# caesar-one/audio-classification-using-a-deep-cnn-combined-with-multi-level-attention

Measured on NVIDIA B200. Metric: 10s-clip audio->logits clips/sec, higher is better.
Workload: dtype fp16

## Files before the change

### audio-classification-using-a-deep-cnn-combined-with-multi-level-attention_b200/b200/_lib.py

```python
from __future__ import annotations

import ctypes as C
import os

_HERE = os.path.dirname(os.path.abspath(__file__))
LIB_PATH = os.environ.get("VMB_LIB") or os.path.join(_HERE, "libvggish_mla_b200.so")

_c_p = C.c_void_p
_ll = C.c_longlong
_int = C.c_int
_sz = C.c_size_t

SIGNATURES = {
    "vmb_last_error": (C.c_char_p, []),
    "vmb_abi_version": (_int, []),
    "vmb_device_arch": (_int, [_int]),
    "vmb_launch_count": (_ll, []),
    "vmb_igemm_pair_enable": (_int, [_int]),
    "vmb_igemm_halo_enable": (_int, [_int]),
    "vmb_mla_fuse_enable": (_int, [_int]),
    "vmb_profile_enable": (_int, [_int]),
    "vmb_profile_collect": (_int, [_c_p, _c_p, _int]),
    "vmb_num_frames": (_ll, [_ll]),
    "vmb_num_examples": (_ll, [_ll]),
    "vmb_logmel": (_int, [_c_p, _ll, _ll, _ll, _ll, _c_p, _c_p]),
    "vmb_logmel_pcm16": (_int, [_c_p, _ll, _ll, _ll, _ll, _c_p, _c_p]),
    "vmb_logmel_cudacore": (_int, [_c_p, _ll, _ll, _ll, _ll, _c_p, _c_p]),
    "vmb_stft_magnitude": (_int, [_c_p, _ll, _c_p, _c_p]),
    "vmb_spec_tiles": (_int, [_c_p, _ll, _int, _int, _int, _c_p, _c_p]),
    "vmb_front_end_tables": (_int, [_c_p, _c_p]),
    "vmb_conv1_relu_pool": (_int, [_c_p, _c_p, _c_p, _c_p, _ll, _c_p]),
    "vmb_conv1_relu_pool_ex": (_int, [_c_p, _c_p, _c_p, _c_p, _ll, _int, _c_p]),
    "vmb_conv1_relu_pool_cudacore": (_int, [_c_p, _c_p, _c_p, _c_p, _ll, _c_p]),
    "vmb_conv3x3_relu": (_int, [_c_p, _c_p, _c_p, _c_p, _ll, _int, _int, _int, _int, _int, _c_p]),
    "vmb_conv3x3_relu_ex": (_int, [_c_p, _c_p, _c_p, _c_p, _ll, _int, _int, _int, _int, _int, _int, _c_p]),
    "vmb_linear_ex": (_int, [_c_p, _c_p, _c_p, _c_p, _int, _int, _ll, _int, _int, _int, _c_p]),
    "vmb_linear": (_int, [_c_p, _c_p, _c_p, _c_p, _int, _int, _ll, _int, _int, _c_p]),
    "vmb_postprocess": (_int, [_c_p, _c_p, _c_p, _c_p, _c_p, _ll, _c_p]),
    "vmb_vggish_create": (_int, [C.POINTER(_c_p), C.POINTER(_c_p), C.POINTER(_c_p), C.POINTER(_c_p),
                                 C.POINTER(_c_p), _c_p]),
    "vmb_vggish_create_ex": (_int, [C.POINTER(_c_p), C.POINTER(_c_p), C.POINTER(_c_p), C.POINTER(_c_p),
                                    C.POINTER(_c_p), _int, _c_p]),
    "vmb_vggish_precision": (_int, [_c_p]),
    "vmb_vggish_saturation": (_int, [_c_p, _int]),
    "vmb_vggish_handle_workspace_bytes": (_sz, [_c_p, _ll]),
    "vmb_vggish_destroy": (None, [_c_p]),
    "vmb_vggish_workspace_bytes": (_sz, [_ll]),
    "vmb_vggish_forward": (_int, [_c_p, _c_p, _ll, _c_p, _c_p, _c_p, _sz, _c_p]),
    "vmb_vggish_fc_train_workspace_bytes": (_sz, [_ll]),
    "vmb_vggish_fc_grad_count": (_ll, []),
    "vmb_vggish_refresh_fc": (_int, [_c_p, C.POINTER(_c_p), C.POINTER(_c_p), _c_p]),
    "vmb_vggish_forward_train": (_int, [_c_p, _c_p, _ll, _c_p, _c_p, _sz, _c_p]),
# ... 79 lines not shown
```

### audio-classification-using-a-deep-cnn-combined-with-multi-level-attention_b200/csrc/api.cu

```cuda
#include "../../include/vggish_mla_b200.h"

#include <cuda_runtime.h>

#include <cstdarg>
#include <cstdio>
#include <cstring>

#include "igemm_sm100.cuh"
#include "kernels.cuh"

namespace {
thread_local char g_api_err[768] = "";

int fail(const char* fmt, ...) {
  va_list ap;
  va_start(ap, fmt);
  vsnprintf(g_api_err, sizeof g_api_err, fmt, ap);
  va_end(ap);
  return 1;
}
int fail_from(const char* where, const char* inner) { return fail("%s: %s", where, inner); }

cudaStream_t S(void* s) { return static_cast<cudaStream_t>(s); }
}

namespace vmb {
void set_api_error(const char* msg) { snprintf(g_api_err, sizeof g_api_err, "%s", msg); }
}

extern "C" {

const char* vmb_last_error(void) { return g_api_err; }
int vmb_abi_version(void) { return 2; }

int vmb_device_arch(int device) {
  int major = 0, minor = 0;
  if (cudaDeviceGetAttribute(&major, cudaDevAttrComputeCapabilityMajor, device) != cudaSuccess ||
      cudaDeviceGetAttribute(&minor, cudaDevAttrComputeCapabilityMinor, device) != cudaSuccess) {
    fail("vmb_device_arch: no CUDA device %d (%s)", device, cudaGetErrorString(cudaGetLastError()));
    return -1;
  }
  return major * 10 + minor;
}

int vmb_igemm_pair_enable(int on) { return vmb::igemm_set_pair(on); }
int vmb_igemm_halo_enable(int on) { return vmb::igemm_set_halo(on); }

long long vmb_num_frames(long long n_samples) {
  const long long d = n_samples - 400;
  long long q = d / 160;
  if (d % 160 != 0 && d < 0) --q;
  return 1 + q;
}

long long vmb_num_examples(long long n_samples) {
  const long long f = vmb_num_frames(n_samples);
  if (f < 96) return f < 0 ? -1 : 0;
  return 1 + (f - 96) / 96;
}

static int logmel_common(const char* who, bool tensor_core, const float* wave, long long n_clips,
                         long long samples_per_clip, long long clip_stride, long long frames_out, float* logmel,
                         void* stream) {
  if (n_clips < 0 || frames_out < 0) return fail("%s: negative size", who);
  const long long nf = vmb_num_frames(samples_per_clip);
  if (nf < 1) return fail("%s: %lld samples is shorter than one 400-sample window", who, samples_per_clip);
  if (frames_out > nf) return fail("%s: frames_out %lld > available frames %lld", who, frames_out, nf);
  if (clip_stride < samples_per_clip) return fail("%s: clip_stride < samples_per_clip", who);
  if (n_clips == 0 || frames_out == 0) return 0;
  if (!wave || !logmel) return fail("%s: null pointer", who);
  const int rc = tensor_core
                     ? vmb::logmel_tc_forward(wave, n_clips, samples_per_clip, clip_stride, frames_out, logmel, S(stream))
                     : vmb::logmel_forward(wave, n_clips, samples_per_clip, clip_stride, frames_out, logmel, S(stream));
  if (rc) return fail_from(who, vmb::kernels_last_error());
  return 0;
}

int vmb_logmel(const float* wave, long long n_clips, long long samples_per_clip, long long clip_stride,
               long long frames_out, float* logmel, void* stream) {
// ... 122 lines not shown
```

### audio-classification-using-a-deep-cnn-combined-with-multi-level-attention_b200/csrc/igemm_sm100.cu

```cuda
#include "igemm_sm100.cuh"

#include <atomic>
#include <cstdio>
#include <cstdlib>
#include <cstring>
#include <mutex>

#include "kernels.cuh"
#include "sm100_ptx.cuh"

namespace vmb {

namespace {

constexpr int kBlockM = 128;
constexpr int kBlockK = 64;
constexpr int kABytes = kBlockM * kBlockK * 2;
constexpr int kQuarterBytes = 32 * kBlockK * 2;
constexpr int kEpiWarps = 8;
constexpr int kEpiThreads = kEpiWarps * 32;
constexpr int kNumThreads = 64 + kEpiThreads;

constexpr int kHaloRows = 10, kHaloWb = 16;
constexpr int kHaloBytes = kHaloRows * kHaloWb * kBlockK * 2;
template <int BLOCK_N, int MT, bool HALO = false>
struct Cfg {
  static constexpr int kBBytes = BLOCK_N * kBlockK * 2;
  static constexpr int kStageBytes = HALO ? MT * kHaloBytes + 3 * kBBytes : MT * kABytes + kBBytes;
  static constexpr int kStages = HALO ? (200 * 1024 / kStageBytes) : ((kStageBytes >= 48 * 1024) ? 4 : 6);
  static_assert(kStages >= 2, "need a double-buffered stage ring");
  static constexpr int kTmemCols = 2 * MT * BLOCK_N;
  static_assert(kTmemCols <= 512, "TMEM holds 512 columns");
  static constexpr int kBiasBytes = 2 * BLOCK_N * 4;
  static constexpr int kBarBytes = (2 * kStages + 4) * 8 + 16;
  static constexpr int kSmemBytes = 1024  + kStages * kStageBytes + kBiasBytes + kBarBytes;
};

constexpr int kOutBf16 = 0, kOutF32 = 1, kOutSplit = 2, kOutF32Atomic = 3;

template <int BLOCK_N, int MT, bool CONV, bool POOL, int OUT, bool BIG = false, bool HALO = false>
__global__ void __launch_bounds__(kNumThreads, 1)
igemm_bf16_kernel(const __grid_constant__ CUtensorMap tmap_a, const __grid_constant__ CUtensorMap tmap_b,
                  const IgemmParams p) {
  static_assert(!HALO || (CONV && BIG && OUT == kOutBf16), "HALO is a variant of the bf16 big-box conv");
  using C = Cfg<BLOCK_N, MT, HALO>;
  extern __shared__ uint8_t smem_raw[];
  uint8_t* smem = reinterpret_cast<uint8_t*>((reinterpret_cast<uintptr_t>(smem_raw) + 1023) & ~uintptr_t(1023));

  uint8_t* stage_base = smem;
  float* bias_s = reinterpret_cast<float*>(smem + C::kStages * C::kStageBytes);
  uint64_t* full_bar = reinterpret_cast<uint64_t*>(smem + C::kStages * C::kStageBytes + C::kBiasBytes);
  uint64_t* empty_bar = full_bar + C::kStages;
  uint64_t* tmem_full = empty_bar + C::kStages;
  uint64_t* tmem_empty = tmem_full + 2;
  uint32_t* tmem_slot = reinterpret_cast<uint32_t*>(tmem_empty + 2);

  const int warp = threadIdx.x >> 5;
  const int lane = threadIdx.x & 31;
  const int mn_tiles = p.num_m_tiles * p.num_n_tiles;
  const int ksplit = p.ksplit > 1 ? p.ksplit : 1;
  const int num_tiles = mn_tiles * ksplit;

  pdl_launch_dependents();
  if (warp == 0 && lane == 0) {
    tma_prefetch_desc(&tmap_a);
    tma_prefetch_desc(&tmap_b);
    for (int s = 0; s < C::kStages; ++s) {
      mbar_init(&full_bar[s], 1);
      mbar_init(&empty_bar[s], 1);
    }
    for (int s = 0; s < 2; ++s) {
      mbar_init(&tmem_full[s], 1);
      mbar_init(&tmem_empty[s], kEpiWarps);
    }
    mbar_fence_init();
  }
  if (warp == 1) tmem_alloc(tmem_slot, C::kTmemCols);
  tc_fence_before_sync();
  __syncthreads();
  tc_fence_after_sync();
  const uint32_t tmem_base = __shfl_sync(0xffffffffu, *tmem_slot, 0);
  pdl_wait();

  if (warp == 0) {
    if (elect_one()) {
      uint32_t stage = 0, phase = 0;
      for (int tile = blockIdx.x; tile < num_tiles; tile += gridDim.x) {
        int mn = tile, kb0 = 0, kb1 = p.num_kb;
        if (ksplit > 1) {
          const int ks = tile / mn_tiles;
          mn = tile - ks * mn_tiles;
          kb0 = p.num_kb * ks / ksplit;
          kb1 = p.num_kb * (ks + 1) / ksplit;
        }
        const int m_tile = mn / p.num_n_tiles;
        const int n_tile = mn - m_tile * p.num_n_tiles;
        int bx[4 * MT], by[4 * MT], bn[4 * MT];
        if (CONV && BIG) {
#pragma unroll
          for (int sub = 0; sub < MT; ++sub) {
            const int g = m_tile * MT + sub;
            const int n_img = g / p.boxes_per_img;
            const int r = g - n_img * p.boxes_per_img;
            const int yy = r / p.boxes_per_row;
            bn[sub] = n_img;
            by[sub] = yy * 4 * p.Hb;
            bx[sub] = (r - yy * p.boxes_per_row) * p.Wb;
          }
        } else if (CONV) {
#pragma unroll
          for (int q = 0; q < 4 * MT; ++q) {
            const int g = m_tile * 4 * MT + q;
            const int n_img = g / p.boxes_per_img;
            const int r = g - n_img * p.boxes_per_img;
            const int yy = r / p.boxes_per_row;
            bn[q] = n_img;
            by[q] = yy * p.Hb;
            bx[q] = (r - yy * p.boxes_per_row) * p.Wb;
          }
        }
        if (HALO) {
          for (int s = 0; s < 3 * p.cblks; ++s) {
            const int cbh = s / 3, dxi = s - cbh * 3;
            mbar_wait(&empty_bar[stage], phase ^ 1);
// ... 48 lines not shown
                            by[q] + dh, bn[q]);
            }
            if (++tap == 9) { tap = 0; ++cb; }
          } else {
            int a_kb = kb;
            if (p.split_nkb) {
              const int q = kb / p.split_nkb;
              const int pa = p.split_planes == 3 ? ((0x210100 >> (4 * (5 - q))) & 0xF) : (q == 1 ? 1 : 0);
              a_kb = pa * p.split_nkb + (kb - q * p.split_nkb);
            }
#pragma unroll
            for (int sub = 0; sub < MT; ++sub)
              tma_load_2d(a_dst + sub * kABytes, &tmap_a, &full_bar[stage], a_kb * kBlockK,
                          (m_tile * MT + sub) * kBlockM);
          }
          int b_kb = CONV ? b_conv_kb : kb;
          if (p.split_nkb) {
            const int q = kb / p.split_nkb;
            const int pb = p.split_planes == 3 ? ((0x012010 >> (4 * (5 - q))) & 0xF) : (q == 2 ? 1 : 0);
            b_kb = pb * p.split_nkb + (kb - q * p.split_nkb);
          }
          tma_load_2d(b_dst, &tmap_b, &full_bar[stage], b_kb * kBlockK, n_tile * BLOCK_N);
          if (++stage == C::kStages) { stage = 0; phase ^= 1; }
        }
      }
    }
  } else if (warp == 1) {
    const uint32_t idesc = p.f16 ? umma_idesc_f16_f32(kBlockM, BLOCK_N) : umma_idesc_bf16_f32(kBlockM, BLOCK_N);
    uint32_t stage = 0, phase = 0, it = 0;
    for (int tile = blockIdx.x; tile < num_tiles; tile += gridDim.x, ++it) {
      const uint32_t acc = it & 1, acc_phase = (it >> 1) & 1;
      int kb0 = 0, kb1 = p.num_kb;
      if (ksplit > 1) {
        const int ks = tile / mn_tiles;
        kb0 = p.num_kb * ks / ksplit;
        kb1 = p.num_kb * (ks + 1) / ksplit;
      }
      mbar_wait(&tmem_empty[acc], acc_phase ^ 1);
      tc_fence_after_sync();
      const uint32_t d_tmem = tmem_base + acc * (MT * BLOCK_N);
      if (HALO) {
        const int n_st = 3 * p.cblks;
        for (int s = 0; s < n_st; ++s) {
          mbar_wait(&full_bar[stage], phase);
          tc_fence_after_sync();
          if (elect_one()) {
            const uint32_t a_addr = smem_u32(stage_base + stage * C::kStageBytes);
            const uint32_t b_addr = a_addr + MT * kHaloBytes;
#pragma unroll
            for (int dyi = 0; dyi < 3; ++dyi) {
              const uint64_t b_desc = umma_desc_kmajor_sw128(b_addr + dyi * C::kBBytes);
#pragma unroll
              for (int sub = 0; sub < MT; ++sub) {
                const uint64_t a_desc = umma_desc_kmajor_sw128(a_addr + sub * kHaloBytes + dyi * (kHaloWb * kBlockK * 2));
#pragma unroll
                for (int k = 0; k < kBlockK / 16; ++k)
                  umma_bf16_ss(d_tmem + sub * BLOCK_N, a_desc + 2 * k, b_desc + 2 * k, idesc, (s | dyi | k) != 0);
              }
            }
            umma_commit(&empty_bar[stage]);
            if (s == n_st - 1) umma_commit(&tmem_full[acc]);
          }
          __syncwarp();
          if (++stage == C::kStages) { stage = 0; phase ^= 1; }
        }
        continue;
      }
      for (int kb = kb0; kb < kb1; ++kb) {
        mbar_wait(&full_bar[stage], phase);
        tc_fence_after_sync();
        if (elect_one()) {
          const uint32_t a_addr = smem_u32(stage_base + stage * C::kStageBytes);
          const uint64_t b_desc = umma_desc_kmajor_sw128(a_addr + MT * kABytes);
#pragma unroll
          for (int sub = 0; sub < MT; ++sub) {
            const uint64_t a_desc = umma_desc_kmajor_sw128(a_addr + sub * kABytes);
#pragma unroll
            for (int k = 0; k < kBlockK / 16; ++k)
              umma_bf16_ss(d_tmem + sub * BLOCK_N, a_desc + 2 * k, b_desc + 2 * k, idesc, ((kb - kb0) | k) != 0);
          }
          umma_commit(&empty_bar[stage]);
          if (kb == kb1 - 1) umma_commit(&tmem_full[acc]);
        }
        __syncwarp();
        if (++stage == C::kStages) { stage = 0; phase ^= 1; }
      }
    }
  } else {
    const int q = warp & 3;
    const int half = (warp - 2) >> 2;
    const int ep_tid = threadIdx.x - 64;
    uint32_t it = 0;
    for (int tile = blockIdx.x; tile < num_tiles; tile += gridDim.x, ++it) {
      int mn = tile, ks = 0;
      if (ksplit > 1) {
        ks = tile / mn_tiles;
        mn = tile - ks * mn_tiles;
      }
      const int m_tile = mn / p.num_n_tiles;
      const int n_tile = mn - m_tile * p.num_n_tiles;
      const int n0 = n_tile * BLOCK_N;
      const uint32_t acc = it & 1, acc_phase = (it >> 1) & 1;
      float* bias_t = bias_s + acc * BLOCK_N;
      for (int i = ep_tid; i < BLOCK_N; i += kEpiThreads)
        bias_t[i] = (p.bias && ks == 0) ? __ldg(p.bias + n0 + i) : 0.f;
      asm volatile("bar.sync 1, %0;" ::"n"(kEpiThreads) : "memory");

      mbar_wait(&tmem_full[acc], acc_phase);
      tc_fence_after_sync();
#pragma unroll 1
      for (int mt = (MT == 2 ? half : 0); mt < (MT == 2 ? half + 1 : 1); ++mt) {
      bool valid;
      size_t out_off;
      int sub = 0;
      if (CONV) {
        const int g = BIG ? (m_tile * MT + mt) : (m_tile * MT + mt) * 4 + q;
        const int n_img = g / p.boxes_per_img;
        const int r = g - n_img * p.boxes_per_img;
        const int yy = r / p.boxes_per_row;
        const int hh = lane / p.Wb, ww = lane - hh * p.Wb;
        const int h = BIG ? yy * 4 * p.Hb + q * p.Hb + hh : yy * p.Hb + hh;
        const int w = (r - yy * p.boxes_per_row) * p.Wb + ww;
        valid = n_img < p.M;
        if (POOL) {
          sub = (ww & 1) | ((hh & 1) << 1);
          out_off = static_cast<size_t>(n_img) * p.out_img_stride +
                    (static_cast<size_t>(h >> 1) * (p.W >> 1) + (w >> 1)) * p.N + n0;
        } else {
          out_off = static_cast<size_t>(n_img) * p.out_img_stride + (static_cast<size_t>(h) * p.W + w) * p.N + n0;
        }
      } else {
        const int row = (m_tile * MT + mt) * kBlockM + q * 32 + lane;
        valid = row < p.M;
        out_off = static_cast<size_t>(row) * p.ldo + n0;
      }

      const uint32_t t_addr = tmem_base + (static_cast<uint32_t>(q * 32) << 16) + acc * (MT * BLOCK_N) + mt * BLOCK_N;
      uint32_t sat_max = 0;

#pragma unroll 1
      for (int ch = (MT == 2 ? 0 : half); ch < BLOCK_N / 32; ch += (MT == 2 ? 1 : 2)) {
        uint32_t v[32];
        tmem_ld_32x32(t_addr + ch * 32, v);
        tmem_ld_wait();
        float f[32];
#pragma unroll
        for (int j = 0; j < 32; j += 4) {
          const float4 b4 = *reinterpret_cast<const float4*>(bias_t + ch * 32 + j);
          f[j + 0] = __uint_as_float(v[j + 0]) + b4.x;
          f[j + 1] = __uint_as_float(v[j + 1]) + b4.y;
          f[j + 2] = __uint_as_float(v[j + 2]) + b4.z;
          f[j + 3] = __uint_as_float(v[j + 3]) + b4.w;
        }
        if (p.relu && !(OUT == kOutBf16 && POOL)) {
#pragma unroll
          for (int j = 0; j < 32; ++j) f[j] = fmaxf(f[j], 0.f);
        }
        if (OUT == kOutSplit) {
          if (POOL) {
#pragma unroll
            for (int j = 0; j < 32; ++j) {
              f[j] = fmaxf(f[j], __shfl_xor_sync(0xffffffffu, f[j], 1));
              f[j] = fmaxf(f[j], __shfl_xor_sync(0xffffffffu, f[j], p.Wb));
            }
          }
          uint32_t hi[16], lo[16];
#pragma unroll
          for (int j = 0; j < 16; ++j) {
            const __nv_bfloat162 h2 = __floats2bfloat162_rn(f[2 * j], f[2 * j + 1]);
            hi[j] = *reinterpret_cast<const uint32_t*>(&h2);
            lo[j] = pack_bf16x2(f[2 * j] - __low2float(h2), f[2 * j + 1] - __high2float(h2));
          }
          __nv_bfloat16* outp = static_cast<__nv_bfloat16*>(p.out) + out_off + ch * 32;
          if (POOL) {
            const bool up = sub & 1;
            if (valid) {
              if (!(sub & 2))
                st_global_256(outp + (up ? 16 : 0), up ? hi[8] : hi[0], up ? hi[9] : hi[1], up ? hi[10] : hi[2],
                              up ? hi[11] : hi[3], up ? hi[12] : hi[4], up ? hi[13] : hi[5], up ? hi[14] : hi[6],
                              up ? hi[15] : hi[7]);
              else
                st_global_256(outp + p.lo_off + (up ? 16 : 0), up ? lo[8] : lo[0], up ? lo[9] : lo[1],
                              up ? lo[10] : lo[2], up ? lo[11] : lo[3], up ? lo[12] : lo[4], up ? lo[13] : lo[5],
                              up ? lo[14] : lo[6], up ? lo[15] : lo[7]);
            }
          } else if (valid) {
            st_global_256(outp, hi[0], hi[1], hi[2], hi[3], hi[4], hi[5], hi[6], hi[7]);
            st_global_256(outp + 16, hi[8], hi[9], hi[10], hi[11], hi[12], hi[13], hi[14], hi[15]);
            st_global_256(outp + p.lo_off, lo[0], lo[1], lo[2], lo[3], lo[4], lo[5], lo[6], lo[7]);
            st_global_256(outp + p.lo_off + 16, lo[8], lo[9], lo[10], lo[11], lo[12], lo[13], lo[14], lo[15]);
          }
        } else if (OUT == kOutF32Atomic) {
          if (valid) {
            float* dst = static_cast<float*>(p.out) + out_off + ch * 32;
#pragma unroll
            for (int j = 0; j < 32; j += 4)
              asm volatile("red.global.v4.f32.add [%0], {%1, %2, %3, %4};" ::"l"(dst + j), "f"(f[j]), "f"(f[j + 1]),
                           "f"(f[j + 2]), "f"(f[j + 3])
                           : "memory");
          }
        } else if (OUT == kOutF32) {
          if (valid) {
            float* dst = static_cast<float*>(p.out) + out_off + ch * 32;
#pragma unroll
            for (int j = 0; j < 32; j += 8)
              st_global_256(dst + j, __float_as_uint(f[j]), __float_as_uint(f[j + 1]), __float_as_uint(f[j + 2]),
                            __float_as_uint(f[j + 3]), __float_as_uint(f[j + 4]), __float_as_uint(f[j + 5]),
                            __float_as_uint(f[j + 6]), __float_as_uint(f[j + 7]));
          }
        } else {
          void* outp = static_cast<uint16_t*>(p.out) + out_off + ch * 32;
          if (p.f16)
            sat_max = max_f16x2(sat_max, store_row32_16bit<true, POOL>(f, sub, p.Wb, p.relu != 0, valid, outp));
          else
            store_row32_16bit<false, POOL>(f, sub, p.Wb, p.relu != 0, valid, outp);
        }
      }
      if (OUT == kOutBf16 && p.f16 && p.sat_flag && saturated_f16x2(sat_max)) *reinterpret_cast<volatile int*>(p.sat_flag) = 1;
      }
      tc_fence_before_sync();
      __syncwarp();
      if (lane == 0) mbar_arrive(&tmem_empty[acc]);
    }
  }

  tc_fence_before_sync();
  __syncthreads();
  if (warp == 1) {
    tc_fence_after_sync();
    tmem_dealloc(tmem_base, C::kTmemCols);
  }
}

thread_local char g_err[512] = "";

bool misaligned32(const void* out, const char* who) {
  if (reinterpret_cast<uintptr_t>(out) % 32 == 0) return false;
  snprintf(g_err, sizeof g_err, "%s: the output buffer must be 32-byte aligned", who);
  return true;
}

using EncodeTiledFn = CUresult (*)(CUtensorMap*, CUtensorMapDataType, cuuint32_t, void*, const cuuint64_t*,
                                   const cuuint64_t*, const cuuint32_t*, const cuuint32_t*, CUtensorMapInterleave,
                                   CUtensorMapSwizzle, CUtensorMapL2promotion, CUtensorMapFloatOOBfill);

EncodeTiledFn get_encode_fn() {
  static EncodeTiledFn fn = nullptr;
  static std::once_flag once;
  std::call_once(once, [] {
    void* ptr = nullptr;
    cudaDriverEntryPointQueryResult qres;
    if (cudaGetDriverEntryPoint("cuTensorMapEncodeTiled", &ptr, cudaEnableDefault, &qres) == cudaSuccess &&
        qres == cudaDriverEntryPointSuccess)
      fn = reinterpret_cast<EncodeTiledFn>(ptr);
  });
// ... 85 lines not shown

const char* igemm_last_error() { return g_err; }

#ifndef VMB_PAIR_DEFAULT
#define VMB_PAIR_DEFAULT 1
#endif
namespace {
std::atomic<int> g_pair_override{-1};
}
bool igemm_use_pair() {
  const int o = g_pair_override.load(std::memory_order_relaxed);
  if (o >= 0) return o != 0;
  static const bool on = [] {
    const char* e = getenv("VMB_IGEMM_PAIR");
    return e ? (e[0] != '0') : (VMB_PAIR_DEFAULT != 0);
  }();
  return on;
}
namespace {
std::atomic<int> g_halo_override{-1};
}
bool igemm_use_halo() {
  const int o = g_halo_override.load(std::memory_order_relaxed);
  if (o >= 0) return o != 0;
  static const bool on = [] {
    const char* e = getenv("VMB_IGEMM_HALO");
    return !(e && e[0] == '0');
  }();
  return on;
}
int igemm_set_halo(int on) {
  const int prev = igemm_use_halo() ? 1 : 0;
  g_halo_override.store(on < 0 ? -1 : (on ? 1 : 0), std::memory_order_relaxed);
  return prev;
}
int igemm_set_pair(int on) {
  const int prev = igemm_use_pair() ? 1 : 0;
  g_pair_override.store(on < 0 ? -1 : (on ? 1 : 0), std::memory_order_relaxed);
  return prev;
}

namespace {
int pair_result(int rc) {
  if (rc) snprintf(g_err, sizeof g_err, "%s", igemm_pair_last_error());
  return rc ? 1 : 0;
}
}

int igemm_linear(const void* a, const void* w, const float* bias, void* out, int out_f32, int relu, int M, int N,
                 int K, cudaStream_t stream, int fmt, int* sat_flag) {
  if (M <= 0) return 0;
  if (misaligned32(out, "igemm_linear")) return 1;
  if (K % kBlockK != 0 || N % 128 != 0) {
    snprintf(g_err, sizeof g_err, "igemm_linear: need K %% 64 == 0 and N %% 128 == 0 (got K=%d N=%d)", K, N);
    return 1;
  }
  if (!out_f32 && N % 256 == 0 && M >= 256 && igemm_use_pair())
    return pair_result(igemm_pair_linear(a, w, bias, out, relu, M, N, K, stream, fmt, sat_flag));
  const int block_n = (N % 256 == 0) ? 256 : 128;
  CUtensorMap ta, tb;
  {
    uint64_t dims[2] = {uint64_t(K), uint64_t(M)};
    uint64_t str[1] = {uint64_t(K) * 2};
    uint32_t box[2] = {kBlockK, kBlockM};
    if (make_tmap_bf16(&ta, a, 2, dims, str, box)) return 1;
  }
// ... 29 lines not shown
  if (K % kBlockK != 0 || N % 128 != 0 || ldo % 16 != 0) {
    snprintf(g_err, sizeof g_err, "igemm_linear_rect: need K %% 64 == 0, N %% 128 == 0, ldo %% 16 == 0");
    return 1;
  }
  CUtensorMap ta, tb;
  {
    uint64_t dims[2] = {uint64_t(K), uint64_t(M)};
    uint64_t str[1] = {uint64_t(K) * 2};
    uint32_t box[2] = {kBlockK, kBlockM};
    if (make_tmap_bf16(&ta, a, 2, dims, str, box)) return 1;
  }
  const int m_tiles = (M + kBlockM - 1) / kBlockM;
  const int block_n = (2 * m_tiles * (N / 128) <= num_sms()) ? 64 : 128;
  {
    uint64_t dims[2] = {uint64_t(K), uint64_t(N)};
    uint64_t str[1] = {uint64_t(K) * 2};
    uint32_t box[2] = {kBlockK, uint32_t(block_n)};
    if (make_tmap_bf16(&tb, w, 2, dims, str, box)) return 1;
  }
  IgemmParams p{};
  p.M = M;
  p.N = N;
  p.num_kb = K / kBlockK;
  p.num_m_tiles = m_tiles;
  p.num_n_tiles = N / block_n;
  p.relu = relu;
  p.ldo = ldo;
  p.bias = bias;
  p.out = out;
  p.f16 = fmt == kFmtF16;
  p.sat_flag = sat_flag;
  return block_n == 64 ? launch<64, 1, false, false, kOutBf16>(ta, tb, p, stream)
                       : launch<128, 1, false, false, kOutBf16>(ta, tb, p, stream);
}

int igemm_linear_split(const void* a_planes, const void* w_planes, const float* bias, float* out, long long ldo,
                       int relu, int M, int N, int K, cudaStream_t stream, int planes) {
  if (M <= 0) return 0;
  if (misaligned32(out, "igemm_linear_split")) return 1;
  if (ldo % 8 != 0) {
    snprintf(g_err, sizeof g_err, "igemm_linear_split: ldo must be a multiple of 8 floats (32-byte rows), got %lld", ldo);
    return 1;
  }
  if (planes != 2 && planes != 3) {
    snprintf(g_err, sizeof g_err, "igemm_linear_split: planes must be 2 or 3");
    return 1;
  }
  if (K % kBlockK != 0 || N % 128 != 0) {
    snprintf(g_err, sizeof g_err, "igemm_linear_split: need K %% 64 == 0 and N %% 128 == 0 (got K=%d N=%d)", K, N);
    return 1;
  }
  if (planes_gemm_enabled()) {
    if (planes_gemm(a_planes, w_planes, bias, out, ldo, relu, M, N, K, planes, 0, stream)) {
      snprintf(g_err, sizeof g_err, "%s", planes_gemm_last_error());
      return 1;
    }
    return 0;
  }
  const int block_n = (N % 256 == 0) ? 256 : 128;
  CUtensorMap ta, tb;
  {
    uint64_t dims[2] = {uint64_t(planes) * K, uint64_t(M)};
    uint64_t str[1] = {uint64_t(planes) * K * 2};
    uint32_t box[2] = {kBlockK, kBlockM};
    if (make_tmap_bf16(&ta, a_planes, 2, dims, str, box)) return 1;
  }
// ... 257 lines not shown
```

### audio-classification-using-a-deep-cnn-combined-with-multi-level-attention_b200/csrc/igemm_sm100.cuh

```cuda
#pragma once
#include <cuda.h>
#include <cuda_runtime.h>
#include <cstdint>

namespace vmb {

struct IgemmParams {
  int M;
  int N;
  int num_kb;
  int cblks;
  int H, W;
  int Hb, Wb;
  int big_box;
  int boxes_per_row;
  int boxes_per_img;
  int total_boxes;
  int num_m_tiles;
  int num_n_tiles;
  int relu;
  int split_nkb;
  int split_planes;
  int ksplit;
  int tile_count;
  int conv_split;
  int f16;
  int* sat_flag;
  long long out_img_stride;
  long long lo_off;
  long long ldo;
  const float* bias;
  void* out;
};

int igemm_linear(const void* a_bf16, const void* w_bf16, const float* bias, void* out, int out_f32, int relu,
                 int M, int N, int K, cudaStream_t stream, int fmt = 0, int* sat_flag = nullptr);
int igemm_linear_split(const void* a_planes, const void* w_planes, const float* bias, float* out, long long ldo,
                       int relu, int M, int N, int K, cudaStream_t stream, int planes = 2);
int igemm_linear_split_ksplit(const void* a_planes, const void* w_planes, float* out_zeroed, long long ldo, int M, int N,
                              int K, cudaStream_t stream, int planes);
int igemm_linear_split_out(const void* a_planes, const void* w_planes, const float* bias, void* out_planes, int relu,
                           int M, int N, int K, cudaStream_t stream);
int igemm_conv3x3_split(const void* act_planes, const void* w_planes, const float* bias, void* out_planes, int n_img,
                        int H, int W, int C_in, int C_out, int pool, cudaStream_t stream);
int igemm_conv3x3(const void* act_bf16, const void* w_bf16, const float* bias, void* out_bf16, int n_img, int H,
                  int W, int C_in, int C_out, int pool, cudaStream_t stream, int fmt = 0, int* sat_flag = nullptr);

int igemm_pair_linear(const void* a_bf16, const void* w_bf16, const float* bias, void* out_bf16, int relu, int M, int N,
                      int K, cudaStream_t stream, int fmt = 0, int* sat_flag = nullptr);
int igemm_pair_conv3x3(const void* act_bf16, const void* w_bf16, const float* bias, void* out_bf16, int n_img, int H,
                       int W, int C_in, int C_out, int pool, cudaStream_t stream, int fmt = 0, int* sat_flag = nullptr);
const char* igemm_pair_last_error();
int igemm_linear_rect(const void* a_bf16, const void* w_bf16, const float* bias, void* out_bf16, long long ldo, int relu,
                         int M, int N, int K, cudaStream_t stream, int fmt = 0, int* sat_flag = nullptr);
bool igemm_use_pair();
int igemm_set_pair(int on);
bool igemm_use_halo();
int igemm_set_halo(int on);

const char* igemm_last_error();

__device__ __forceinline__ float dropout_scale(unsigned long long seed, unsigned layer, unsigned long long idx, float p) {
  if (p <= 0.f) return 1.f;
  const unsigned key = static_cast<unsigned>(seed) ^ (static_cast<unsigned>(seed >> 32) * 0x9E3779B1u) ^
                       (layer * 0x85EBCA77u + 0xC2B2AE3Du);
  unsigned h = (static_cast<unsigned>(idx) ^ key) * 0x9E3779B1u + static_cast<unsigned>(idx >> 32) * 0x27D4EB2Fu;
  h ^= h >> 16;
  h *= 0x85EBCA6Bu;
  h ^= h >> 13;
  h *= 0xC2B2AE35u;
  h ^= h >> 16;
  const float u = static_cast<float>(h >> 8) * (1.0f / 16777216.0f);
  return u >= p ? 1.f / (1.f - p) : 0.f;
}

int planes_gemm(const void* a_planes, const void* b_planes, const float* bias, float* out, long long ldo, int relu, int M,
                int N, int K, int planes, int ksplit, cudaStream_t stream);
struct PlanesEpi {
  int mode;
  int T, relu, cols, cpad;
  const float *a1, *b1, *a2, *b2;
  void *dst, *dst2;
};
int planes_gemm_fused(const void* a_planes, const void* b_planes, const float* bias, const PlanesEpi& epi, int M, int N,
                      int K, cudaStream_t stream);
struct PlanesStats {
  double* acc;
  float* stat;
  unsigned* counter;
  float *run_mean, *run_var;
  double count;
// ... 31 lines not shown
```

### audio-classification-using-a-deep-cnn-combined-with-multi-level-attention_b200/csrc/vggish.cu

```cuda
#include <cuda_bf16.h>

#include <cstdio>
#include <cstring>
#include <string>

#include "../../include/vggish_mla_b200.h"
#include "fc_train.cuh"
#include "igemm_sm100.cuh"
#include "kernels.cuh"

namespace vmb {
void set_api_error(const char* msg);
}

struct HostStage {
  cudaStream_t copy_st = nullptr;
  cudaEvent_t wave_ready[2] = {}, wave_free[2] = {};
  void* d_wave[2] = {};
  size_t wave_cap[2] = {};
  unsigned long long batches = 0;
  void* d_ws = nullptr;
  size_t ws_cap = 0;
  float* d_scores[2] = {};
  size_t scores_cap[2] = {};
  cudaEvent_t done[2] = {};
  bool busy[2] = {false, false};
  unsigned long long calls = 0;
};

struct vmb_vggish {
  int precision = 0;
  bool has_fc = true;
  int* sat = nullptr;
  float* conv1_w = nullptr;
  float* conv_b[6] = {};
  void* conv_w[6] = {};
  void* fc_w[3] = {};
  float* fc_b[3] = {};
  void* train_w[3] = {};
  void* train_wt[3] = {};
  HostStage stage;
};

namespace {

struct ConvGeom { int H, W, C_in, C_out, pool; };
constexpr ConvGeom kConv[5] = {{48, 32, 64, 128, 1}, {24, 16, 128, 256, 0}, {24, 16, 256, 256, 1},
                               {12, 8, 256, 512, 0}, {12, 8, 512, 512, 1}};
constexpr int kFcIn[3] = {12288, 4096, 4096};
constexpr int kFcOut[3] = {4096, 4096, 128};
constexpr size_t kBufA = 196608;
constexpr size_t kBufB = 98304;

int fail(const char* fmt, const char* detail = "") {
  char buf[640];
  snprintf(buf, sizeof buf, fmt, detail);
  vmb::set_api_error(buf);
  return 1;
}

size_t align_up(size_t v, size_t a) { return (v + a - 1) / a * a; }

bool fc_inference_copy(vmb_vggish* h, int i, const float* w, const float* b, cudaStream_t st) {
  if (cudaMemcpyAsync(h->fc_b[i], b, size_t(kFcOut[i]) * 4, cudaMemcpyDeviceToDevice, st) != cudaSuccess) return false;
  const int fmt = h->precision == 2 ? 1 : 0;
  return (h->precision == 1 ? vmb::split_f32_to_planes(w, h->fc_w[i], kFcOut[i], kFcIn[i], st)
                            : vmb::cast_f32_to_bf16(w, h->fc_w[i], static_cast<long long>(kFcOut[i]) * kFcIn[i], st,
                                                    fmt)) == 0;
}

char* conv_stack(vmb_vggish* h, const float* examples, long long n, void* workspace, cudaStream_t st, const char* who) {
  const bool split = h->precision == 1;
  const int fmt = h->precision == 2 ? 1 : 0;
  int* sat = h->sat;
  const size_t mul = split ? 2 : 1;
  char* A = static_cast<char*>(workspace);
  char* B = A + align_up(size_t(n) * kBufA * mul, 1024);
  {
    vmb::StageTimer t(VMB_STAGE_CONV1, st);
    if (vmb::conv1_tc_relu_pool(examples, h->conv1_w, h->conv_b[0], A, n, st, split, fmt, sat)) {
      fail("%s", (std::string(who) + ": " + vmb::kernels_last_error()).c_str());
      return nullptr;
    }
  }
  char* src = A;
// ... 33 lines not shown
    if (!conv_w[i] || !conv_b[i]) return fail("vmb_vggish_create: null conv tensor");
  for (int i = 0; i < 3 && has_fc; ++i)
    if (!fc_w[i] || !fc_b[i]) return fail("vmb_vggish_create: null fc tensor");
  cudaStream_t st = static_cast<cudaStream_t>(stream);
  vmb_vggish* h = new vmb_vggish();
  h->precision = precision;
  h->has_fc = has_fc;
  const size_t wmul = precision == 1 ? 2 : 1;
  const int fmt = precision == 2 ? 1 : 0;
  bool ok = true;
  if (precision == 2) {
    ok = cudaHostAlloc(reinterpret_cast<void**>(&h->sat), 8 * sizeof(int), cudaHostAllocMapped) == cudaSuccess;
    if (ok) memset(h->sat, 0, 8 * sizeof(int));
  }
  auto dmalloc = [&](void** p, size_t bytes) { ok = ok && cudaMalloc(p, bytes) == cudaSuccess; };
  auto dcopy = [&](void* d, const void* s, size_t bytes) {
    ok = ok && cudaMemcpyAsync(d, s, bytes, cudaMemcpyDeviceToDevice, st) == cudaSuccess;
  };
  dmalloc(reinterpret_cast<void**>(&h->conv1_w), 64 * 9 * 4);
  dmalloc(reinterpret_cast<void**>(&h->conv_b[0]), 64 * 4);
  if (ok) {
    dcopy(h->conv1_w, conv_w[0], 64 * 9 * 4);
    dcopy(h->conv_b[0], conv_b[0], 64 * 4);
  }
  for (int i = 0; i < 5 && ok; ++i) {
    const ConvGeom& g = kConv[i];
    dmalloc(&h->conv_w[i + 1], size_t(g.C_out) * 9 * g.C_in * 2 * wmul);
    dmalloc(reinterpret_cast<void**>(&h->conv_b[i + 1]), size_t(g.C_out) * 4);
    if (!ok) break;
    dcopy(h->conv_b[i + 1], conv_b[i + 1], size_t(g.C_out) * 4);
    ok = ok && (precision == 1 ? vmb::relayout_conv_weight_split(conv_w[i + 1], h->conv_w[i + 1], g.C_out, g.C_in, st)
                               : vmb::relayout_conv_weight(conv_w[i + 1], h->conv_w[i + 1], g.C_out, g.C_in, st, fmt)) == 0;
  }
  for (int i = 0; i < 3 && ok && has_fc; ++i) {
    dmalloc(&h->fc_w[i], size_t(kFcOut[i]) * kFcIn[i] * 2 * wmul);
    dmalloc(reinterpret_cast<void**>(&h->fc_b[i]), size_t(kFcOut[i]) * 4);
    if (!ok) break;
    ok = ok && fc_inference_copy(h, i, fc_w[i], fc_b[i], st);
  }
  ok = ok && cudaStreamSynchronize(st) == cudaSuccess;
  if (!ok) {
    const char* why = cudaGetErrorString(cudaGetLastError());
    vmb_vggish_destroy(h);
    return fail("vmb_vggish_create: allocation / re-layout failed (%s)", why);
  }
  *handle = h;
  return 0;
}

void vmb_vggish_destroy(vmb_vggish_t* h) {
  if (!h) return;
  cudaFree(h->conv1_w);
  for (int i = 0; i < 6; ++i) {
    cudaFree(h->conv_b[i]);
    cudaFree(h->conv_w[i]);
  }
  for (int i = 0; i < 3; ++i) {
    cudaFree(h->fc_w[i]);
    cudaFree(h->fc_b[i]);
    cudaFree(h->train_w[i]);
    cudaFree(h->train_wt[i]);
  }
  if (h->sat) cudaFreeHost(h->sat);
  HostStage& hs = h->stage;
  for (int i = 0; i < 2; ++i) {
    cudaFree(hs.d_wave[i]);
    cudaFree(hs.d_scores[i]);
    if (hs.wave_ready[i]) cudaEventDestroy(hs.wave_ready[i]);
    if (hs.wave_free[i]) cudaEventDestroy(hs.wave_free[i]);
    if (hs.done[i]) cudaEventDestroy(hs.done[i]);
  }
  cudaFree(hs.d_ws);
  if (hs.copy_st) cudaStreamDestroy(hs.copy_st);
  delete h;
}

size_t vmb_vggish_workspace_bytes(long long n) {
  if (n <= 0) return 0;
  return align_up(size_t(n) * kBufA, 1024) + align_up(size_t(n) * kBufB, 1024);
}

size_t vmb_vggish_handle_workspace_bytes(const vmb_vggish_t* h, long long n) {
  if (n <= 0 || !h) return 0;
  const size_t mul = h->precision == 1 ? 2 : 1;
  return align_up(size_t(n) * kBufA * mul, 1024) + align_up(size_t(n) * kBufB * mul, 1024);
}

int vmb_vggish_precision(const vmb_vggish_t* h) { return h ? h->precision : -1; }

int vmb_vggish_saturation(vmb_vggish_t* h, int clear) {
  if (!h || !h->sat) return 0;
  int mask = 0;
  for (int i = 0; i < 8; ++i) {
    if (*reinterpret_cast<volatile int*>(h->sat + i)) mask |= 1 << i;
    if (clear) h->sat[i] = 0;
  }
  return mask;
}

int vmb_vggish_forward(vmb_vggish_t* h, const float* examples, long long n, float* emb, void* bottleneck,
                       void* workspace, size_t workspace_bytes, void* stream) {
  if (!h) return fail("vmb_vggish_forward: null handle");
  if (n < 0) return fail("vmb_vggish_forward: negative n");
  if (n == 0) return 0;
  if (n > 1000000) return fail("vmb_vggish_forward: at most 1 000 000 examples per call (chunk on the host)");
  if (!examples || !workspace || (!emb && !bottleneck)) return fail("vmb_vggish_forward: null pointer");
  if (emb && !h->has_fc) return fail("vmb_vggish_forward: this handle was built without the FC stack (bottleneck features only)");
  if (workspace_bytes < vmb_vggish_handle_workspace_bytes(h, n)) return fail("vmb_vggish_forward: workspace too small");
  if (reinterpret_cast<uintptr_t>(workspace) % 1024) return fail("vmb_vggish_forward: workspace must be 1024-byte aligned");
  cudaStream_t st = static_cast<cudaStream_t>(stream);
  const bool split = h->precision == 1;
  const int fmt = h->precision == 2 ? 1 : 0;
  int* sat = h->sat;
  const size_t mul = split ? 2 : 1;
  char* A = static_cast<char*>(workspace);
  char* B = A + align_up(size_t(n) * kBufA * mul, 1024);
  char* src = conv_stack(h, examples, n, workspace, st, "vmb_vggish_forward");
  if (!src) return 1;
  char* dst = src == A ? B : A;
  if (bottleneck) {
    const cudaError_t e = split
        ? cudaMemcpy2DAsync(bottleneck, size_t(12288) * 2, src, size_t(2) * 12288 * 2, size_t(12288) * 2, size_t(n),
                            cudaMemcpyDeviceToDevice, st)
        : cudaMemcpyAsync(bottleneck, src, size_t(n) * 12288 * 2, cudaMemcpyDeviceToDevice, st);
    if (e != cudaSuccess) return fail("vmb_vggish_forward: bottleneck copy failed");
  }
  if (!emb) return 0;
  const void* fc_in[3] = {src, dst, src};
  void* fc_out[3] = {dst, src, emb};
  for (int i = 0; i < 3; ++i) {
    vmb::StageTimer t(VMB_STAGE_FC1 + i, st);
    int rc;
    if (!split)
      rc = vmb::igemm_linear(fc_in[i], h->fc_w[i], h->fc_b[i], fc_out[i], i == 2, 1, int(n), kFcOut[i], kFcIn[i], st, fmt,
                             (sat && i < 2) ? sat + 6 + i : nullptr);
    else if (i < 2)
      rc = vmb::igemm_linear_split_out(fc_in[i], h->fc_w[i], h->fc_b[i], fc_out[i], 1, int(n), kFcOut[i], kFcIn[i], st);
    else
      rc = vmb::igemm_linear_split(fc_in[i], h->fc_w[i], h->fc_b[i], emb, kFcOut[i], 1, int(n), kFcOut[i], kFcIn[i], st);
    if (rc) return fail("vmb_vggish_forward: %s", vmb::igemm_last_error());
  }
  return 0;
}

namespace {
vmb::FcTrainLayout train_layout(long long n) { return vmb::fc_train_layout(n, vmb_vggish_workspace_bytes(n) * 2); }

int check_train_args(const vmb_vggish_t* h, long long n, const void* ws, size_t ws_bytes, const char* who) {
  char msg[256];
  auto bad = [&](const char* why) {
    snprintf(msg, sizeof msg, "%s: %s", who, why);
    return fail("%s", msg);
  };
  if (!h) return bad("null handle");
  if (!h->has_fc) return bad("this handle was built without the FC stack (bottleneck features only)");
  if (!h->train_w[0]) return bad("no training copy of the FC weights: call vmb_vggish_refresh_fc first");
  if (n < 1) return bad("n must be at least 1");
  if (n > 1000000) return bad("at most 1 000 000 examples per call");
  if (!ws) return bad("null workspace");
  if (reinterpret_cast<uintptr_t>(ws) % 1024) return bad("workspace must be 1024-byte aligned");
  if (ws_bytes < train_layout(n).total) return bad("workspace too small for n examples");
  return 0;
}
}

extern "C" {
// ... 256 lines not shown
```

### include/vggish_mla_b200.h

```cpp
#ifndef VGGISH_MLA_B200_H_
#define VGGISH_MLA_B200_H_

#include <stddef.h>
#include <stdint.h>

#ifdef __cplusplus
extern "C" {
#endif

typedef struct vmb_vggish vmb_vggish_t;
typedef struct vmb_mla vmb_mla_t;
typedef struct vmb_mla_trainer vmb_mla_trainer_t;

const char* vmb_last_error(void);
int vmb_abi_version(void);
int vmb_device_arch(int device);

long long vmb_launch_count(void);
int vmb_igemm_pair_enable(int on);
int vmb_igemm_halo_enable(int on);
int vmb_mla_fuse_enable(int on);
enum {
  VMB_STAGE_LOGMEL = 0, VMB_STAGE_CONV1 = 1, VMB_STAGE_CONV2 = 2, VMB_STAGE_CONV3_1 = 3, VMB_STAGE_CONV3_2 = 4,
  VMB_STAGE_CONV4_1 = 5, VMB_STAGE_CONV4_2 = 6, VMB_STAGE_FC1 = 7, VMB_STAGE_FC2 = 8, VMB_STAGE_FC3 = 9,
  VMB_STAGE_MLA = 10, VMB_STAGE_POSTPROCESS = 11, VMB_NUM_STAGES = 12
};
int vmb_profile_enable(int on);
int vmb_profile_collect(double* ms_per_stage, long long* calls_per_stage, int reset);


long long vmb_num_frames(long long n_samples);
long long vmb_num_examples(long long n_samples);

int vmb_logmel(const float* wave_dev, long long n_clips, long long samples_per_clip, long long clip_stride,
               long long frames_out, float* logmel_dev, void* stream);

int vmb_logmel_pcm16(const int16_t* pcm_dev, long long n_clips, long long samples_per_clip, long long clip_stride,
                     long long frames_out, float* logmel_dev, void* stream);

int vmb_stft_magnitude(const double* signal_dev, long long n_samples, double* mag_dev, void* stream);

int vmb_logmel_cudacore(const float* wave_dev, long long n_clips, long long samples_per_clip, long long clip_stride,
                        long long frames_out, float* logmel_dev, void* stream);

int vmb_spec_tiles(const float* examples_dev, long long n_clips, int n_examples_per_clip, int n_frames, int overlap,
                   float* out_dev, void* stream);

int vmb_front_end_tables(double* hann400, double* mel257x64);


int vmb_conv1_relu_pool(const float* examples_dev, const float* w_dev, const float* b_dev, void* out_bf16_dev,
                        long long n, void* stream);
int vmb_conv1_relu_pool_ex(const float* examples_dev, const float* w_dev, const float* b_dev, void* out_16bit_dev,
// ... 108 lines not shown
```

Baseline: 72780.

## Split-K the FC3 GEMM with per-slice partials and last-CTA reduction

FC3 (4096->128) has very few output tiles, so it runs a split-K kernel with seven K slices. Each slice writes fp32 partials into a scratch buffer, and a per-tile atomic counter lets the last-arriving CTA sum the slices and apply bias and ReLU. The aim is to fill more SMs on a narrow-N GEMM. In exchange it adds partial-buffer traffic and threadfence/counter synchronisation, and it changes the k-split tile ordering used by existing split-K paths.

```diff
diff --git a/audio-classification-using-a-deep-cnn-combined-with-multi-level-attention_b200/b200/_lib.py b/audio-classification-using-a-deep-cnn-combined-with-multi-level-attention_b200/b200/_lib.py
--- a/audio-classification-using-a-deep-cnn-combined-with-multi-level-attention_b200/b200/_lib.py
+++ b/audio-classification-using-a-deep-cnn-combined-with-multi-level-attention_b200/b200/_lib.py
@@ -18,6 +18,7 @@
     "vmb_launch_count": (_ll, []),
     "vmb_igemm_pair_enable": (_int, [_int]),
     "vmb_igemm_halo_enable": (_int, [_int]),
+    "vmb_fc_slices_enable": (_int, [_int]),
     "vmb_mla_fuse_enable": (_int, [_int]),
     "vmb_profile_enable": (_int, [_int]),
     "vmb_profile_collect": (_int, [_c_p, _c_p, _int]),
diff --git a/audio-classification-using-a-deep-cnn-combined-with-multi-level-attention_b200/csrc/api.cu b/audio-classification-using-a-deep-cnn-combined-with-multi-level-attention_b200/csrc/api.cu
--- a/audio-classification-using-a-deep-cnn-combined-with-multi-level-attention_b200/csrc/api.cu
+++ b/audio-classification-using-a-deep-cnn-combined-with-multi-level-attention_b200/csrc/api.cu
@@ -45,6 +45,7 @@
 
 int vmb_igemm_pair_enable(int on) { return vmb::igemm_set_pair(on); }
 int vmb_igemm_halo_enable(int on) { return vmb::igemm_set_halo(on); }
+int vmb_fc_slices_enable(int on) { return vmb::fc_slices_set(on); }
 
 long long vmb_num_frames(long long n_samples) {
   const long long d = n_samples - 400;
diff --git a/audio-classification-using-a-deep-cnn-combined-with-multi-level-attention_b200/csrc/igemm_sm100.cu b/audio-classification-using-a-deep-cnn-combined-with-multi-level-attention_b200/csrc/igemm_sm100.cu
--- a/audio-classification-using-a-deep-cnn-combined-with-multi-level-attention_b200/csrc/igemm_sm100.cu
+++ b/audio-classification-using-a-deep-cnn-combined-with-multi-level-attention_b200/csrc/igemm_sm100.cu
@@ -36,7 +36,9 @@
   static constexpr int kSmemBytes = 1024  + kStages * kStageBytes + kBiasBytes + kBarBytes;
 };
 
-constexpr int kOutBf16 = 0, kOutF32 = 1, kOutSplit = 2, kOutF32Atomic = 3;
+constexpr int kMaxSlices = 8;
+constexpr int kOutBf16 = 0, kOutF32 = 1, kOutSplit = 2, kOutF32Atomic = 3,
+              kOutF32Slices = 4;
 
 template <int BLOCK_N, int MT, bool CONV, bool POOL, int OUT, bool BIG = false, bool HALO = false>
 __global__ void __launch_bounds__(kNumThreads, 1)
@@ -88,8 +90,8 @@
       for (int tile = blockIdx.x; tile < num_tiles; tile += gridDim.x) {
         int mn = tile, kb0 = 0, kb1 = p.num_kb;
         if (ksplit > 1) {
-          const int ks = tile / mn_tiles;
-          mn = tile - ks * mn_tiles;
+          mn = tile / ksplit;
+          const int ks = tile - mn * ksplit;
           kb0 = p.num_kb * ks / ksplit;
           kb1 = p.num_kb * (ks + 1) / ksplit;
         }
@@ -204,7 +206,7 @@
       const uint32_t acc = it & 1, acc_phase = (it >> 1) & 1;
       int kb0 = 0, kb1 = p.num_kb;
       if (ksplit > 1) {
-        const int ks = tile / mn_tiles;
+        const int ks = tile % ksplit;
         kb0 = p.num_kb * ks / ksplit;
         kb1 = p.num_kb * (ks + 1) / ksplit;
       }
@@ -266,8 +268,8 @@
     for (int tile = blockIdx.x; tile < num_tiles; tile += gridDim.x, ++it) {
       int mn = tile, ks = 0;
       if (ksplit > 1) {
-        ks = tile / mn_tiles;
-        mn = tile - ks * mn_tiles;
+        mn = tile / ksplit;
+        ks = tile - mn * ksplit;
       }
       const int m_tile = mn / p.num_n_tiles;
       const int n_tile = mn - m_tile * p.num_n_tiles;
@@ -275,7 +277,7 @@
       const uint32_t acc = it & 1, acc_phase = (it >> 1) & 1;
       float* bias_t = bias_s + acc * BLOCK_N;
       for (int i = ep_tid; i < BLOCK_N; i += kEpiThreads)
-        bias_t[i] = (p.bias && ks == 0) ? __ldg(p.bias + n0 + i) : 0.f;
+        bias_t[i] = (p.bias && ks == 0 && OUT != kOutF32Slices) ? __ldg(p.bias + n0 + i) : 0.f;
       asm volatile("bar.sync 1, %0;" ::"n"(kEpiThreads) : "memory");
 
       mbar_wait(&tmem_full[acc], acc_phase);
@@ -304,7 +306,8 @@
       } else {
         const int row = (m_tile * MT + mt) * kBlockM + q * 32 + lane;
         valid = row < p.M;
-        out_off = static_cast<size_t>(row) * p.ldo + n0;
+        out_off = OUT == kOutF32Slices ? (static_cast<size_t>(ks) * p.M + row) * p.N + n0
+                                       : static_cast<size_t>(row) * p.ldo + n0;
       }
 
       const uint32_t t_addr = tmem_base + (static_cast<uint32_t>(q * 32) << 16) + acc * (MT * BLOCK_N) + mt * BLOCK_N;
@@ -324,7 +327,7 @@
           f[j + 2] = __uint_as_float(v[j + 2]) + b4.z;
           f[j + 3] = __uint_as_float(v[j + 3]) + b4.w;
         }
-        if (p.relu && !(OUT == kOutBf16 && POOL)) {
+        if (p.relu && !(OUT == kOutBf16 && POOL) && OUT != kOutF32Slices) {
 #pragma unroll
           for (int j = 0; j < 32; ++j) f[j] = fmaxf(f[j], 0.f);
         }
@@ -371,9 +374,9 @@
                            "f"(f[j + 2]), "f"(f[j + 3])
                            : "memory");
           }
-        } else if (OUT == kOutF32) {
+        } else if (OUT == kOutF32 || OUT == kOutF32Slices) {
           if (valid) {
-            float* dst = static_cast<float*>(p.out) + out_off + ch * 32;
+            float* dst = (OUT == kOutF32Slices ? p.partial : static_cast<float*>(p.out)) + out_off + ch * 32;
 #pragma unroll
             for (int j = 0; j < 32; j += 8)
               st_global_256(dst + j, __float_as_uint(f[j]), __float_as_uint(f[j + 1]), __float_as_uint(f[j + 2]),
@@ -393,6 +396,66 @@
       tc_fence_before_sync();
       __syncwarp();
       if (lane == 0) mbar_arrive(&tmem_empty[acc]);
+      if (OUT == kOutF32Slices) {
+        volatile uint32_t* last_s = tmem_slot + 1;
+        __threadfence();
+        asm volatile("bar.sync 1, %0;" ::"n"(kEpiThreads) : "memory");
+        if (ep_tid == 0) {
+          const unsigned arrived = atomicAdd(p.tile_cnt + mn, 1u);
+          *last_s = arrived == static_cast<unsigned>(ksplit - 1);
+          if (arrived == static_cast<unsigned>(ksplit - 1)) p.tile_cnt[mn] = 0u;
+        }
+        asm volatile("bar.sync 1, %0;" ::"n"(kEpiThreads) : "memory");
+        if (*last_s) {
+          __threadfence();
+          const int r0 = m_tile * kBlockM;
+          const int rows = p.M - r0 < kBlockM ? p.M - r0 : kBlockM;
+          constexpr int kV = BLOCK_N / 4;
+          constexpr int kU = 2;
+          const size_t slice = static_cast<size_t>(p.M) * p.N;
+          const int n_vec = rows * kV;
+          for (int i0 = ep_tid; i0 < n_vec; i0 += kU * kEpiThreads) {
+            float4 t[kU][kMaxSlices];
+#pragma unroll
+            for (int u = 0; u < kU; ++u) {
+              const int i = i0 + u * kEpiThreads, r = i / kV;
+              const size_t off = static_cast<size_t>(r0 + r) * p.N + n0 + (i - r * kV) * 4;
+#pragma unroll
+              for (int k = 0; k < kMaxSlices; ++k)
+                if (i < n_vec && k < ksplit) t[u][k] = __ldcg(reinterpret_cast<const float4*>(p.partial + k * slice + off));
+            }
+#pragma unroll
+            for (int u = 0; u < kU; ++u) {
+              const int i = i0 + u * kEpiThreads, r = i / kV, c = n0 + (i - r * kV) * 4;
+              if (i >= n_vec) break;
+              float4 s = t[u][0];
+#pragma unroll
+              for (int k = 1; k < kMaxSlices; ++k) {
+                if (k < ksplit) {
+                  s.x += t[u][k].x;
+                  s.y += t[u][k].y;
+                  s.z += t[u][k].z;
+                  s.w += t[u][k].w;
+                }
+              }
+              if (p.bias) {
+                const float4 b4 = __ldg(reinterpret_cast<const float4*>(p.bias + c));
+                s.x += b4.x;
+                s.y += b4.y;
+                s.z += b4.z;
+                s.w += b4.w;
+              }
+              if (p.relu) {
+                s.x = fmaxf(s.x, 0.f);
+                s.y = fmaxf(s.y, 0.f);
+                s.z = fmaxf(s.z, 0.f);
+                s.w = fmaxf(s.w, 0.f);
+              }
+              *reinterpret_cast<float4*>(static_cast<float*>(p.out) + static_cast<size_t>(r0 + r) * p.ldo + c) = s;
+            }
+          }
+        }
+      }
     }
   }
 
@@ -544,6 +607,23 @@
 int igemm_set_halo(int on) {
   const int prev = igemm_use_halo() ? 1 : 0;
   g_halo_override.store(on < 0 ? -1 : (on ? 1 : 0), std::memory_order_relaxed);
+  return prev;
+}
+namespace {
+std::atomic<int> g_slices_override{-1};
+}
+bool fc_slices_enabled() {
+  const int o = g_slices_override.load(std::memory_order_relaxed);
+  if (o >= 0) return o != 0;
+  static const bool on = [] {
+    const char* e = getenv("VMB_FC_SLICES");
+    return !(e && e[0] == '0');
+  }();
+  return on;
+}
+int fc_slices_set(int on) {
+  const int prev = fc_slices_enabled() ? 1 : 0;
+  g_slices_override.store(on < 0 ? -1 : (on ? 1 : 0), std::memory_order_relaxed);
   return prev;
 }
 int igemm_set_pair(int on) {
@@ -639,6 +719,46 @@
   p.sat_flag = sat_flag;
   return block_n == 64 ? launch<64, 1, false, false, kOutBf16>(ta, tb, p, stream)
                        : launch<128, 1, false, false, kOutBf16>(ta, tb, p, stream);
+}
+
+int igemm_linear_slices(const void* a, const void* w, const float* bias, float* out, int relu, int M, int N, int K,
+                        int slices, float* partial, unsigned* tile_cnt, cudaStream_t stream, int fmt) {
+  if (M <= 0) return 0;
+  if (misaligned32(out, "igemm_linear_slices") || misaligned32(partial, "igemm_linear_slices (partials)")) return 1;
+  if (K % kBlockK != 0 || N % 128 != 0 || slices < 2 || slices > kMaxSlices || K / kBlockK < slices || !tile_cnt) {
+    snprintf(g_err, sizeof g_err,
+             "igemm_linear_slices: need K %% 64 == 0, N %% 128 == 0, 2 <= slices <= min(8, K / 64) and counters (K=%d N=%d S=%d)",
+             K, N, slices);
+    return 1;
+  }
+  CUtensorMap ta, tb;
+  {
+    uint64_t dims[2] = {uint64_t(K), uint64_t(M)};
+    uint64_t str[1] = {uint64_t(K) * 2};
+    uint32_t box[2] = {kBlockK, kBlockM};
+    if (make_tmap_bf16(&ta, a, 2, dims, str, box)) return 1;
+  }
+  {
+    uint64_t dims[2] = {uint64_t(K), uint64_t(N)};
+    uint64_t str[1] = {uint64_t(K) * 2};
+    uint32_t box[2] = {kBlockK, 128};
+    if (make_tmap_bf16(&tb, w, 2, dims, str, box)) return 1;
+  }
+  IgemmParams p{};
+  p.M = M;
+  p.N = N;
+  p.num_kb = K / kBlockK;
+  p.num_m_tiles = (M + kBlockM - 1) / kBlockM;
+  p.num_n_tiles = N / 128;
+  p.ksplit = slices;
+  p.relu = relu;
+  p.ldo = N;
+  p.bias = bias;
+  p.out = out;
+  p.partial = partial;
+  p.tile_cnt = tile_cnt;
+  p.f16 = fmt == kFmtF16;
+  return launch<128, 1, false, false, kOutF32Slices>(ta, tb, p, stream);
 }
 
 int igemm_linear_split(const void* a_planes, const void* w_planes, const float* bias, float* out, long long ldo,
diff --git a/audio-classification-using-a-deep-cnn-combined-with-multi-level-attention_b200/csrc/igemm_sm100.cuh b/audio-classification-using-a-deep-cnn-combined-with-multi-level-attention_b200/csrc/igemm_sm100.cuh
--- a/audio-classification-using-a-deep-cnn-combined-with-multi-level-attention_b200/csrc/igemm_sm100.cuh
+++ b/audio-classification-using-a-deep-cnn-combined-with-multi-level-attention_b200/csrc/igemm_sm100.cuh
@@ -31,10 +31,14 @@
   long long ldo;
   const float* bias;
   void* out;
+  float* partial;
+  unsigned* tile_cnt;
 };
 
 int igemm_linear(const void* a_bf16, const void* w_bf16, const float* bias, void* out, int out_f32, int relu,
                  int M, int N, int K, cudaStream_t stream, int fmt = 0, int* sat_flag = nullptr);
+int igemm_linear_slices(const void* a, const void* w, const float* bias, float* out, int relu, int M, int N, int K,
+                        int slices, float* partial, unsigned* tile_cnt, cudaStream_t stream, int fmt = 0);
 int igemm_linear_split(const void* a_planes, const void* w_planes, const float* bias, float* out, long long ldo,
                        int relu, int M, int N, int K, cudaStream_t stream, int planes = 2);
 int igemm_linear_split_ksplit(const void* a_planes, const void* w_planes, float* out_zeroed, long long ldo, int M, int N,
@@ -57,6 +61,8 @@
 int igemm_set_pair(int on);
 bool igemm_use_halo();
 int igemm_set_halo(int on);
+bool fc_slices_enabled();
+int fc_slices_set(int on);
 
 const char* igemm_last_error();
 
diff --git a/audio-classification-using-a-deep-cnn-combined-with-multi-level-attention_b200/csrc/vggish.cu b/audio-classification-using-a-deep-cnn-combined-with-multi-level-attention_b200/csrc/vggish.cu
--- a/audio-classification-using-a-deep-cnn-combined-with-multi-level-attention_b200/csrc/vggish.cu
+++ b/audio-classification-using-a-deep-cnn-combined-with-multi-level-attention_b200/csrc/vggish.cu
@@ -37,6 +37,7 @@
   void* conv_w[6] = {};
   void* fc_w[3] = {};
   float* fc_b[3] = {};
+  unsigned* fc3_cnt = nullptr;
   void* train_w[3] = {};
   void* train_wt[3] = {};
   HostStage stage;
@@ -51,6 +52,8 @@
 constexpr int kFcOut[3] = {4096, 4096, 128};
 constexpr size_t kBufA = 196608;
 constexpr size_t kBufB = 98304;
+constexpr int kFc3Slices = 7;
+constexpr long long kMaxExamples = 1000000;
 
 int fail(const char* fmt, const char* detail = "") {
   char buf[640];
@@ -150,6 +153,11 @@
     ok = ok && (precision == 1 ? vmb::relayout_conv_weight_split(conv_w[i + 1], h->conv_w[i + 1], g.C_out, g.C_in, st)
                                : vmb::relayout_conv_weight(conv_w[i + 1], h->conv_w[i + 1], g.C_out, g.C_in, st, fmt)) == 0;
   }
+  if (has_fc && precision != 1) {
+    const size_t cnt_bytes = size_t((kMaxExamples + 127) / 128) * (kFcOut[2] / 128) * sizeof(unsigned);
+    dmalloc(reinterpret_cast<void**>(&h->fc3_cnt), cnt_bytes);
+    ok = ok && cudaMemsetAsync(h->fc3_cnt, 0, cnt_bytes, st) == cudaSuccess;
+  }
   for (int i = 0; i < 3 && ok && has_fc; ++i) {
     dmalloc(&h->fc_w[i], size_t(kFcOut[i]) * kFcIn[i] * 2 * wmul);
     dmalloc(reinterpret_cast<void**>(&h->fc_b[i]), size_t(kFcOut[i]) * 4);
@@ -179,6 +187,7 @@
     cudaFree(h->train_w[i]);
     cudaFree(h->train_wt[i]);
   }
+  cudaFree(h->fc3_cnt);
   if (h->sat) cudaFreeHost(h->sat);
   HostStage& hs = h->stage;
   for (int i = 0; i < 2; ++i) {
@@ -221,7 +230,7 @@
   if (!h) return fail("vmb_vggish_forward: null handle");
   if (n < 0) return fail("vmb_vggish_forward: negative n");
   if (n == 0) return 0;
-  if (n > 1000000) return fail("vmb_vggish_forward: at most 1 000 000 examples per call (chunk on the host)");
+  if (n > kMaxExamples) return fail("vmb_vggish_forward: at most 1 000 000 examples per call (chunk on the host)");
   if (!examples || !workspace || (!emb && !bottleneck)) return fail("vmb_vggish_forward: null pointer");
   if (emb && !h->has_fc) return fail("vmb_vggish_forward: this handle was built without the FC stack (bottleneck features only)");
   if (workspace_bytes < vmb_vggish_handle_workspace_bytes(h, n)) return fail("vmb_vggish_forward: workspace too small");
@@ -249,7 +258,10 @@
   for (int i = 0; i < 3; ++i) {
     vmb::StageTimer t(VMB_STAGE_FC1 + i, st);
     int rc;
-    if (!split)
+    if (!split && i == 2 && vmb::fc_slices_enabled())
+      rc = vmb::igemm_linear_slices(fc_in[i], h->fc_w[i], h->fc_b[i], emb, 1, int(n), kFcOut[i], kFcIn[i], kFc3Slices,
+                                    reinterpret_cast<float*>(dst), h->fc3_cnt, st, fmt);
+    else if (!split)
       rc = vmb::igemm_linear(fc_in[i], h->fc_w[i], h->fc_b[i], fc_out[i], i == 2, 1, int(n), kFcOut[i], kFcIn[i], st, fmt,
                              (sat && i < 2) ? sat + 6 + i : nullptr);
     else if (i < 2)
diff --git a/include/vggish_mla_b200.h b/include/vggish_mla_b200.h
--- a/include/vggish_mla_b200.h
+++ b/include/vggish_mla_b200.h
@@ -19,6 +19,7 @@
 long long vmb_launch_count(void);
 int vmb_igemm_pair_enable(int on);
 int vmb_igemm_halo_enable(int on);
+int vmb_fc_slices_enable(int on);
 int vmb_mla_fuse_enable(int on);
 enum {
   VMB_STAGE_LOGMEL = 0, VMB_STAGE_CONV1 = 1, VMB_STAGE_CONV2 = 2, VMB_STAGE_CONV3_1 = 3, VMB_STAGE_CONV3_2 = 4,
```

Result: no change. 72380 (median of 6 runs) (-0.6%).
